# bede/kindel

Hardware: NVIDIA H100
Metric: aligned bases/sec through pileup+consensus (higher is better)
Workload: dtype int32

## Files before the change

kindel_b200/csrc/api.cu:

```cuda
#include <atomic>
#include <cstdio>
#include <cstdlib>
#include <cstring>
#include <new>

#include "kdl_common.cuh"
#include "pileup_general.cu"
#include "pileup_simple.cu"
#include "pileup_tile.cu"
#include "pileup_mask.cu"
#include "vote.cu"
#include "assemble.cu"
#include "variants.cu"
#include "select.cu"
#include "primers.cu"
#include "mates.cu"
#include "quality.cu"
#include "amplicons.cu"
#include "normalise.cu"
#include "dedup.cu"
#include "left_align.cu"

namespace {

// ... 31 lines not shown
    static std::atomic<int> done[kMaxDevices];
    const int dev = current_device();
    if (done[dev].load(std::memory_order_acquire)) return KDL_OK;
    if (cudaFuncSetAttribute(kdl::pileup_tile_kernel<kFlush, kCx>, cudaFuncAttributeMaxDynamicSharedMemorySize,
                             (int)sizeof(kdl::TileSmem<kdl::TileCfg<kCx>>)) != cudaSuccess)
        return KDL_ERR_CUDA;
    done[dev].store(1, std::memory_order_release);
    return KDL_OK;
}

inline int check_launch() {
    g_launches.fetch_add(1, std::memory_order_relaxed);
    return cudaGetLastError() == cudaSuccess ? KDL_OK : KDL_ERR_CUDA;
}
#else
inline int sm_count() { return emu::M().sm_count; }

template <int kFlush, bool kCx>
inline int ensure_tile_smem() { return KDL_OK; }

inline int check_launch() {
    g_launches.fetch_add(1, std::memory_order_relaxed);
    return emu::take_launch_error() ? KDL_ERR_CUDA : KDL_OK;
}
#endif

template <int kFlush, bool kCx>
inline int launch_tile(const kdl_batch& b, int32_t* counts, long long n_slots, long long tile_lo, long long n_tiles,
                       int split, int zero_rest, uint32_t* dirty_map, uint32_t map_after, cudaStream_t st) {
    int rc = ensure_tile_smem<kFlush, kCx>();
    if (rc != KDL_OK) return rc;
    const long long units = n_tiles * split, max_grid = (long long)sm_count() * 2;
    const long long grid = units < max_grid ? units : max_grid;
    KDL_LAUNCH((kdl::pileup_tile_kernel<kFlush, kCx>), (unsigned)grid, kdl::W_THREADS,
               sizeof(kdl::TileSmem<kdl::TileCfg<kCx>>), st,
               b, counts, n_slots, b.tile_index, tile_lo, n_tiles, split, zero_rest, dirty_map, map_after);
    return KDL_OK;
}

int depth_split(long long units, int per_sm, long long reads) {
    int split = 1;
    const long long slots = (long long)sm_count() * per_sm;
    if (units < slots) {
        long long want = (slots + units - 1) / units;
        const long long deep = reads / (units * 256);
        if (want > deep) want = deep;
        split = (int)(want < 1 ? 1 : (want > 32 ? 32 : want));
    }
    if (const char* ev = getenv("KDL_SPLIT")) { const int v = atoi(ev); if (v >= 1 && v <= 64) split = v; }
    return split;
}

int validate_batch(const kdl_batch* b) {
    if (!b || b->n_reads < 0 || b->n_contigs < 0 || b->n_hard < 0 || b->n_complex < b->n_hard)
        return KDL_ERR_INVALID_ARG;
    if (b->n_reads > 0 && (!b->ref_start || !b->seq_off || !b->l_seq || !b->seq4 ||
                           !b->contig_read_off || !b->contig_len || !b->contig_slot))
        return KDL_ERR_INVALID_ARG;
    if ((b->n_hard > 0 && !b->hard_idx) || (b->n_complex > 0 && !b->complex_idx)) return KDL_ERR_INVALID_ARG;
    if (b->reach_right < b->max_simple_len || b->reach_left < 0) return KDL_ERR_INVALID_ARG;
    return KDL_OK;
}

}

extern "C" {

int kdl_abi_version(void) { return KDL_ABI_VERSION; }

const char* kdl_status_string(int status) {
    switch (status) {
        case KDL_OK: return "ok";
        case KDL_ERR_INVALID_ARG: return "invalid argument";
        case KDL_ERR_CUDA: return "CUDA error";
        case KDL_ERR_NO_DEVICE: return "no CUDA device";
        case KDL_ERR_INDEX: return "IndexError: read walks off the contig or off its SEQ";
        case KDL_ERR_KEY: return "KeyError: base outside A,C,G,T,N in an M or S op";
        default: return "unknown status";
    }
}

int64_t kdl_launch_count(void) { return g_launches.load(std::memory_order_relaxed); }

int kdl_pileup(const kdl_batch* batch, int32_t* counts, int64_t n_slots, int32_t* ins_events,
               int32_t* err_flag, void* stream) {
    return kdl_pileup_range(batch, counts, n_slots, 0, n_slots, 0, ins_events, err_flag, stream);
}

int kdl_pileup_range(const kdl_batch* batch, int32_t* counts, int64_t n_slots, int64_t slot_lo,
                     int64_t slot_hi, int32_t flags, int32_t* ins_events, int32_t* err_flag, void* stream) {
    return kdl_pileup_range_map(batch, counts, n_slots, slot_lo, slot_hi, flags, nullptr, ins_events, err_flag, stream);
}

int kdl_pileup_range_map(const kdl_batch* batch, int32_t* counts, int64_t n_slots, int64_t slot_lo, int64_t slot_hi,
                         int32_t flags, uint32_t* dirty_map, int32_t* ins_events, int32_t* err_flag, void* stream) {
    int rc = validate_batch(batch);
    if (rc != KDL_OK) return rc;
    if (!counts || !err_flag || n_slots <= 0 || slot_lo < 0 || slot_hi > n_slots || slot_lo > slot_hi ||
        (reinterpret_cast<uintptr_t>(dirty_map) & 15))
        return KDL_ERR_INVALID_ARG;
    const bool tileable = (n_slots % KDL_TILE) == 0 && (slot_lo % KDL_TILE) == 0 && (slot_hi % KDL_TILE) == 0;
    if ((slot_lo & 3) || (slot_hi & 3)) return KDL_ERR_INVALID_ARG;
    cudaStream_t st = (cudaStream_t)stream;
    const int cap = sm_count() * 8;
    const bool has_tile_reads = batch->n_reads > batch->n_hard;
    const bool tiled = has_tile_reads && tileable && batch->reads_sorted && batch->tile_index &&
                       batch->reach_right > 0 && batch->reach_right <= KDL_FAST_MAXLEN + KDL_TILE_MAXREACH;
    const bool fresh = (flags & KDL_PILEUP_FRESH_WEIGHTS) != 0;
    const long long tile_lo = slot_lo / KDL_TILE, n_tiles = (slot_hi - slot_lo) / KDL_TILE;
    const int split = tiled && n_tiles > 0 ? depth_split(n_tiles, 2, batch->n_reads) : 1;
    bool cx_by_atomics = (batch->n_complex - batch->n_hard) * 16 < batch->n_reads;
    if (const char* ev = getenv("KDL_CX")) cx_by_atomics = !strcmp(ev, "atomics") ? true : (!strcmp(ev, "pieces") ? false : cx_by_atomics);
    const int zero_in_k1 = (tiled && split == 1 && fresh && n_tiles > 0 && (flags & KDL_PILEUP_ZERO_REST)) ? 1 : 0;
    const int zero_from = (fresh && !(tiled && split == 1)) ? 0 : 5;
    const int zero_to = ((flags & KDL_PILEUP_ZERO_REST) && !zero_in_k1) ? KDL_NCOL : 5;
    const bool zero_pass = zero_to > zero_from && slot_hi > slot_lo;
    const bool k1_stores = tiled && split == 1 && fresh && n_tiles > 0;
    const bool saturate = dirty_map && batch->n_complex > 0 && batch->n_complex * 16 >= batch->n_reads &&
                          (k1_stores || zero_pass);
    uint32_t* mark_map = saturate ? nullptr : dirty_map;
    if (zero_pass) {
        uint32_t* zmap = saturate || (zero_from <= 5 && zero_to == KDL_NCOL) ? dirty_map : nullptr;
        KDL_LAUNCH(kdl::zero_cols_kernel, sm_count() * 4, 256, 0, st, counts, n_slots, zero_from, zero_to, slot_lo,
                   slot_hi, zmap, saturate ? ~0u : 0u);
        if ((rc = check_launch()) != KDL_OK) return rc;
    }
    const uint32_t map_after = saturate && k1_stores ? ~0u : 0u;
    if (batch->n_reads == 0) return KDL_OK;
    if (tiled) {
        if (n_tiles > 0) {
            KDL_LAUNCH(kdl::tile_index_kernel, (unsigned)((n_tiles * 32 + 255) / 256), 256, 0, st, *batch, tile_lo,
                       n_tiles, batch->tile_index);
            if ((rc = check_launch()) != KDL_OK) return rc;
            const bool cx = batch->n_complex > batch->n_hard && !cx_by_atomics;
            if (split > 1) {
                rc = cx ? launch_tile<kdl::F_ATOMIC, true>(*batch, counts, n_slots, tile_lo, n_tiles, split, 0, nullptr, 0, st)
                        : launch_tile<kdl::F_ATOMIC, false>(*batch, counts, n_slots, tile_lo, n_tiles, split, 0, nullptr, 0, st);
            } else if (fresh) {
                rc = cx ? launch_tile<kdl::F_STORE, true>(*batch, counts, n_slots, tile_lo, n_tiles, 1, zero_in_k1, dirty_map,
                                                          map_after, st)
                        : launch_tile<kdl::F_STORE, false>(*batch, counts, n_slots, tile_lo, n_tiles, 1, zero_in_k1, dirty_map,
                                                           map_after, st);
            } else {
                rc = cx ? launch_tile<kdl::F_ADD, true>(*batch, counts, n_slots, tile_lo, n_tiles, 1, 0, nullptr, 0, st)
                        : launch_tile<kdl::F_ADD, false>(*batch, counts, n_slots, tile_lo, n_tiles, 1, 0, nullptr, 0, st);
            }
            if (rc != KDL_OK) return rc;
            if ((rc = check_launch()) != KDL_OK) return rc;
        }
        if (batch->n_complex > batch->n_hard && cx_by_atomics && n_tiles > 0) {
            const long long n_win = (slot_hi - slot_lo + kdl::CW_SLOTS - 1) / kdl::CW_SLOTS;
            const int wsplit = depth_split(n_win, 8, batch->n_complex - batch->n_hard);
            KDL_LAUNCH(kdl::pileup_window_kernel, (unsigned)(n_win * wsplit), kdl::CW_THREADS,
                       sizeof(int32_t) * kdl::CW_SMEM_COLS * kdl::CW_SLOTS, st, *batch, counts, n_slots, slot_lo,
                       slot_hi, wsplit, ins_events, mark_map);
            if ((rc = check_launch()) != KDL_OK) return rc;
        } else if (batch->n_complex > batch->n_hard && !cx_by_atomics) {
            KDL_LAUNCH(kdl::pileup_events_kernel, (unsigned)((batch->n_complex + 255) / 256), 256, 0, st, *batch, counts,
                       n_slots, ins_events, mark_map);
            if ((rc = check_launch()) != KDL_OK) return rc;
        }
        if (batch->n_hard > 0) {
            const int grid = grid_for(batch->n_hard, 8, cap);
            KDL_LAUNCH(kdl::pileup_general_kernel, grid, 256, 0, st, *batch, batch->hard_idx, batch->n_hard, counts,
                       n_slots, ins_events, err_flag, mark_map);
            if ((rc = check_launch()) != KDL_OK) return rc;
        }
    } else {
        if (batch->n_reads > batch->n_complex) {
            const int grid = grid_for(batch->n_reads, 8, cap);
            KDL_LAUNCH(kdl::pileup_simple_atomic_kernel, grid, 256, 0, st, *batch, counts, n_slots, err_flag);
            if ((rc = check_launch()) != KDL_OK) return rc;
        }
        if (batch->n_complex > 0) {
            const int grid = grid_for(batch->n_reads, 8, cap);
            KDL_LAUNCH(kdl::pileup_general_kernel, grid, 256, 0, st, *batch, nullptr, batch->n_reads, counts, n_slots,
                       ins_events, err_flag, mark_map);
            if ((rc = check_launch()) != KDL_OK) return rc;
        }
    }
    return KDL_OK;
}

int kdl_unmask(const kdl_batch* batch, const kdl_qmask* qmask, int32_t* counts, int64_t n_slots, void* stream) {
    int rc = validate_batch(batch);
    if (rc != KDL_OK) return rc;
    if (!qmask || !counts || n_slots <= 0 || qmask->n_reads < 0 || qmask->n_bases < 0 || qmask->n_reads > batch->n_reads)
        return KDL_ERR_INVALID_ARG;
    if (qmask->n_reads == 0) return KDL_OK;
    if (!qmask->read_idx || !qmask->off || !qmask->qpos) return KDL_ERR_INVALID_ARG;
    const long long grid = (qmask->n_reads + kdl::kQThreads - 1) / kdl::kQThreads;
    KDL_LAUNCH(kdl::unmask_kernel, (unsigned)grid, kdl::kQThreads, 0, (cudaStream_t)stream, *batch, *qmask, counts,
               n_slots);
    return check_launch();
}

int kdl_diagnose(const kdl_batch* batch, kdl_diag* diag_dev, void* stream) {
    int rc = validate_batch(batch);
    if (rc != KDL_OK) return rc;
    if (!diag_dev) return KDL_ERR_INVALID_ARG;
    cudaStream_t st = (cudaStream_t)stream;
    KDL_LAUNCH(kdl::diagnose_init_kernel, 1, 1, 0, st, diag_dev);
    if ((rc = check_launch()) != KDL_OK) return rc;
    if (batch->n_hard > 0) {
        const long long grid = (batch->n_hard + 255) / 256;
        KDL_LAUNCH(kdl::diagnose_kernel, (unsigned)grid, 256, 0, st, *batch, diag_dev);
        if ((rc = check_launch()) != KDL_OK) return rc;
    }
    KDL_LAUNCH(kdl::diagnose_final_kernel, 1, 1, 0, st, diag_dev);
    return check_launch();
}

int kdl_vote(const int32_t* counts, int64_t n_slots, int64_t min_depth_ceil, uint8_t* calls,
             void* stream) {
    if (!counts || !calls || n_slots <= 0 || (n_slots & 3)) return KDL_ERR_INVALID_ARG;
    kdl::Peers none;
    none.n = 0;
    const long long quads = n_slots / 4;
    const long long grid = (quads + 255) / 256;
    KDL_LAUNCH(kdl::vote_kernel<false>, (unsigned)grid, 256, 0, (cudaStream_t)stream,
               counts, none, n_slots, 0, n_slots, min_depth_ceil, calls, nullptr, kdl::MajorityVote{});
    return check_launch();
}

static bool valid_threshold(double t) { return t >= 0.0 && t <= 1.0; }

int kdl_vote_iupac(const int32_t* counts, int64_t n_slots, int64_t min_depth_ceil, double threshold, uint8_t* calls,
                   void* stream) {
    if (!counts || !calls || n_slots <= 0 || (n_slots & 3) || !valid_threshold(threshold)) return KDL_ERR_INVALID_ARG;
    kdl::Peers none;
    none.n = 0;
    const long long quads = n_slots / 4;
    const long long grid = (quads + 255) / 256;
    KDL_LAUNCH((kdl::vote_kernel<false, kdl::IupacVote>), (unsigned)grid, 256, 0, (cudaStream_t)stream,
               counts, none, n_slots, 0, n_slots, min_depth_ceil, calls, nullptr, kdl::IupacVote{threshold});
    return check_launch();
}

int kdl_derive(const int32_t* counts, int64_t n_slots, int32_t* out, void* stream) {
    if (!counts || !out || n_slots <= 0) return KDL_ERR_INVALID_ARG;
    const long long grid = (n_slots + 255) / 256;
    KDL_LAUNCH(kdl::derive_kernel, (unsigned)grid, 256, 0, (cudaStream_t)stream, counts, n_slots, out);
    return check_launch();
}

int kdl_vote_peers(const int32_t* const* peer_counts, int32_t n_peers, int64_t n_slots,
                   int64_t slot_lo, int64_t slot_hi, int64_t min_depth_ceil, uint8_t* calls,
                   int32_t* reduced, void* stream) {
    return kdl_vote_peers_sparse(peer_counts, nullptr, nullptr, n_peers, n_slots, slot_lo, slot_hi,
                                 min_depth_ceil, calls, reduced, stream);
}

static int make_exchange(const kdl_exchange* x, kdl::Exchange* e, int64_t n_slots) {
    if (!x || x->n_ranks < 1 || x->n_ranks > 16 || x->rank < 0 || x->rank >= x->n_ranks || !x->counter)
        return KDL_ERR_INVALID_ARG;
    e->peers.n = x->n_ranks;
    e->rank = x->rank;
    e->counter = x->counter;
    for (int p = 0; p < x->n_ranks; ++p) {
        if (!x->tables[p] || !x->calls[p] || !x->ready[p] || !x->done[p]) return KDL_ERR_INVALID_ARG;
        e->peers.tab[p] = x->tables[p];
        e->peers.lo[p] = x->foot_lo[p];
        e->peers.hi[p] = n_slots > 0 && x->foot_hi[p] > n_slots ? n_slots : x->foot_hi[p];
        if ((e->peers.lo[p] & 3) || (e->peers.hi[p] & 3)) return KDL_ERR_INVALID_ARG;
        e->calls[p] = x->calls[p];
        e->ready[p] = x->ready[p];
        e->done[p] = x->done[p];
        e->slice_lo[p] = x->slice_lo[p];
        e->slice_hi[p] = x->slice_hi[p];
        if ((x->slice_lo[p] & 3) || (x->slice_hi[p] & 3) || x->slice_hi[p] < x->slice_lo[p]) return KDL_ERR_INVALID_ARG;
    }
    e->ready_local = x->ready[x->rank];
    e->done_local = x->done[x->rank];
    return KDL_OK;
}

int kdl_exchange_signal(const kdl_exchange* x, int32_t epoch, void* stream) {
    kdl::Exchange e;
    int rc = make_exchange(x, &e, 0);
    if (rc != KDL_OK) return rc;
    KDL_LAUNCH(kdl::exchange_signal_kernel, 1, 32, 0, (cudaStream_t)stream, e, epoch);
    return check_launch();
}

int kdl_exchange_wait(const kdl_exchange* x, int32_t epoch, void* stream) {
    kdl::Exchange e;
    int rc = make_exchange(x, &e, 0);
    if (rc != KDL_OK) return rc;
    dim3 grid((unsigned)(sm_count() * 2 / x->n_ranks + 1), (unsigned)x->n_ranks);
    KDL_LAUNCH(kdl::exchange_gather_kernel, grid, 256, 0, (cudaStream_t)stream, e, epoch);
    return check_launch();
}

extern "C++" template <class Vote>
int exchange_vote(const kdl_exchange* x, int64_t n_slots, int64_t min_depth_ceil, int32_t epoch, Vote vote,
                  void* stream) {
    if (n_slots <= 0 || (n_slots & 3)) return KDL_ERR_INVALID_ARG;
    kdl::Exchange e;
    int rc = make_exchange(x, &e, n_slots);
    if (rc != KDL_OK) return rc;
    if (x->slice_hi[x->rank] > n_slots) return KDL_ERR_INVALID_ARG;
    const long long quads = (x->slice_hi[x->rank] - x->slice_lo[x->rank]) / 4;
    long long grid = (quads + 255) / 256;
    const long long cap = (long long)sm_count() * 8;
    if (grid > cap) grid = cap;
    if (grid < 1) grid = 1;
    KDL_LAUNCH(kdl::vote_exchange_kernel<Vote>, (unsigned)grid, 256, 0, (cudaStream_t)stream, e, n_slots,
// ... 698 lines not shown
```

kindel_b200/csrc/pileup_general.cu:

```cuda
#include "tile_common.cuh"

namespace kdl {

__global__ void __launch_bounds__(256)
pileup_general_kernel(kdl_batch b, const uint32_t* __restrict__ list, long long n_list, int32_t* __restrict__ counts,
                      long long n_slots, int32_t* __restrict__ ins_events, int32_t* __restrict__ err_flag,
                      uint32_t* __restrict__ dirty_map = nullptr) {
    const int lane = threadIdx.x & 31;
    const bool marks = dirty_map != nullptr && lane == 0;
    const long long warp0 = ((long long)blockIdx.x * blockDim.x + threadIdx.x) >> 5;
    const long long n_warps = ((long long)gridDim.x * blockDim.x) >> 5;
    bool bad = false;

    for (long long j = warp0; j < n_list; j += n_warps) {
        const long long r = list ? (long long)list[j] : j;
        const uint32_t lraw = (uint32_t)b.l_seq[r];
        if (!(lraw & KDL_COMPLEX)) continue;
        const int c = find_contig(b.contig_read_off, b.n_contigs, r);
        const long long L = b.contig_len[c];
        const long long base = b.contig_slot[c];
        const long long lseq = complex_len(lraw);
        const uint32_t* __restrict__ seq = b.seq4 + (size_t)b.seq_off[r];
        const uint32_t* __restrict__ blk = seq + ((lseq + 7) >> 3);
        const uint32_t c0 = 0, c1 = blk[0];
// ... 9 lines not shown
            if (op == 0 || op == 7 || op == 8) {
                for (long long k = lane; k < len; k += 32) {
                    const long long q = q_pos + k;
                    const long long idx = pyindex(r_pos + k, L);
                    if (q >= lseq || idx < 0) { bad = true; continue; }
                    const int col = nib2col(nibble_at(seq, q));
                    if (col < 0) { bad = true; continue; }
                    atomicAdd(counts + (long long)(KDL_W_A + col) * n_slots + base + idx, 1);
                }
                r_pos += len;
                q_pos += len;
            } else if (op == 1) {
                if (marks) mark_dirty_py(dirty_map, KDL_INS, 1, base, r_pos, r_pos + 1, L + 1);
                if (lane == 0) {
                    const long long idx = pyindex(r_pos, L + 1);
                    if (idx < 0) {
                        bad = true;
                    } else {
                        atomicAdd(counts + (long long)KDL_INS * n_slots + base + idx, 1);
                        if (ins_events) {
                            int4 e = make_int4((int)(base + idx), (int)r, (int)q_pos, (int)len);
                            reinterpret_cast<int4*>(ins_events)[evt] = e;
                        }
                    }
                }
                evt += 1;
                q_pos += len;
            } else if (op == 2) {
                if (marks) mark_dirty_py(dirty_map, KDL_DEL, 1, base, r_pos, r_pos + len, L + 1);
                for (long long k = lane; k < len; k += 32) {
                    const long long idx = pyindex(r_pos + k, L + 1);
                    if (idx < 0) { bad = true; continue; }
                    atomicAdd(counts + (long long)KDL_DEL * n_slots + base + idx, 1);
                }
                r_pos += len;
            } else if (op == 4) {
                if (i == c0) {
                    if (marks) {
                        mark_dirty_py(dirty_map, KDL_CLIP_ENDS, 1, base, r_pos, r_pos + 1, L + 1);
                        mark_dirty(dirty_map, KDL_CEW_A, 5, base + (r_pos - len > 0 ? r_pos - len : 0),
                                   base + (r_pos < L ? r_pos : L));
                    }
                    if (lane == 0) {
                        const long long idx = pyindex(r_pos, L + 1);
                        if (idx < 0) bad = true;
                        else atomicAdd(counts + (long long)KDL_CLIP_ENDS * n_slots + base + idx, 1);
                    }
                    for (long long g = lane; g < len; g += 32) {
                        if (g >= lseq) { bad = true; continue; }
                        const long long rel = r_pos - len + g;
                        if (rel < 0) continue;
                        if (rel >= L) { bad = true; continue; }
                        const int col = nib2col(nibble_at(seq, g));
                        if (col < 0) { bad = true; continue; }
                        atomicAdd(counts + (long long)(KDL_CEW_A + col) * n_slots + base + rel, 1);
                    }
                    q_pos += len;
                } else {
                    if (lane == 0) {
                        const long long idx = pyindex(r_pos - 1, L + 1);
                        if (idx < 0) bad = true;
                        else atomicAdd(counts + (long long)KDL_CLIP_STARTS * n_slots + base + idx, 1);
                    }
                    long long n_adv = L - r_pos;
                    n_adv = n_adv < 0 ? 0 : (n_adv > len ? len : n_adv);
                    if (marks) {
                        mark_dirty_py(dirty_map, KDL_CLIP_STARTS, 1, base, r_pos - 1, r_pos, L + 1);
                        mark_dirty_py(dirty_map, KDL_CSW_A, 5, base, r_pos, r_pos + n_adv, L);
                    }
                    for (long long k = lane; k < n_adv; k += 32) {
                        const long long q = q_pos + k;
                        const long long idx = pyindex(r_pos + k, L);
                        if (q >= lseq || idx < 0) { bad = true; continue; }
                        const int col = nib2col(nibble_at(seq, q));
                        if (col < 0) { bad = true; continue; }
                        atomicAdd(counts + (long long)(KDL_CSW_A + col) * n_slots + base + idx, 1);
                    }
                    if (n_adv < len && q_pos + n_adv >= lseq) bad = true;
                    r_pos += n_adv;
                    q_pos += n_adv;
                }
            }
        }
    }
    if (bad) atomicOr(err_flag, 1);
}

__global__ void __launch_bounds__(256)
pileup_events_kernel(kdl_batch b, int32_t* __restrict__ counts, long long n_slots, int32_t* __restrict__ ins_events,
                     uint32_t* __restrict__ dirty_map) {
    const long long j = (long long)blockIdx.x * blockDim.x + threadIdx.x;
    if (j >= b.n_complex) return;
    const long long r = (long long)b.complex_idx[j];
    const uint32_t lraw = (uint32_t)b.l_seq[r];
    if ((lraw & (KDL_COMPLEX | KDL_HARD)) != KDL_COMPLEX) return;
    const int c = find_contig(b.contig_read_off, b.n_contigs, r);
    const long long slot0 = b.contig_slot[c];
    int32_t* __restrict__ tab = counts + slot0;
    const uint32_t* __restrict__ seq = b.seq4 + (size_t)b.seq_off[r];
    const uint32_t* __restrict__ blk = seq + (((lraw & KDL_LEN_MASK) + 7) >> 3);
    const int n_ops = (int)blk[0];
    uint32_t evt = blk[1];
    const uint32_t* __restrict__ ops = blk + 2;
    long long r_pos = b.ref_start[r];
    int q_pos = 0;
    for (int o = 0; o < n_ops; ++o) {
        const uint32_t cg = ops[o];
        const int len = (int)(cg >> 4);
        const int op = (int)(cg & 0xF);
        if (op == 0 || op == 7 || op == 8) {
            r_pos += len;
            q_pos += len;
        } else if (op == 1) {
            if (dirty_map) mark_dirty(dirty_map, KDL_INS, 1, slot0 + r_pos, slot0 + r_pos + 1);
            atomicAdd(tab + (long long)KDL_INS * n_slots + r_pos, 1);
            if (ins_events)
                reinterpret_cast<int4*>(ins_events)[evt] = make_int4((int)(slot0 + r_pos), (int)r, q_pos, len);
            evt += 1;
            q_pos += len;
        } else if (op == 2) {
            if (dirty_map) mark_dirty(dirty_map, KDL_DEL, 1, slot0 + r_pos, slot0 + r_pos + len);
            for (int d = 0; d < len; ++d) atomicAdd(tab + (long long)KDL_DEL * n_slots + r_pos + d, 1);
            r_pos += len;
        } else if (op == 4) {
            if (o == 0) {
                if (dirty_map) {
                    mark_dirty(dirty_map, KDL_CLIP_ENDS, 1, slot0 + r_pos, slot0 + r_pos + 1);
                    mark_dirty(dirty_map, KDL_CEW_A, 5, slot0 + (r_pos - len > 0 ? r_pos - len : 0), slot0 + r_pos);
                }
                atomicAdd(tab + (long long)KDL_CLIP_ENDS * n_slots + r_pos, 1);
                for (int g = 0; g < len; ++g) {
                    const long long rel = r_pos - len + g;
                    if (rel >= 0) atomicAdd(tab + (long long)(KDL_CEW_A + nib2col(nibble_at(seq, g))) * n_slots + rel, 1);
                }
                q_pos += len;
            } else {
                if (dirty_map) {
                    mark_dirty(dirty_map, KDL_CLIP_STARTS, 1, slot0 + r_pos - 1, slot0 + r_pos);
                    mark_dirty(dirty_map, KDL_CSW_A, 5, slot0 + r_pos, slot0 + r_pos + len);
                }
                atomicAdd(tab + (long long)KDL_CLIP_STARTS * n_slots + r_pos - 1, 1);
                for (int d = 0; d < len; ++d)
                    atomicAdd(tab + (long long)(KDL_CSW_A + nib2col(nibble_at(seq, q_pos + d))) * n_slots + r_pos + d, 1);
                r_pos += len;
                q_pos += len;
            }
        }
    }
}

constexpr int CW_SLOTS = 1024;
constexpr int CW_THREADS = 256;
constexpr int CW_SMEM_COLS = 7;
static_assert(CW_SLOTS % KDL_TILE == 0 && CW_SLOTS % 256 == 0, "windows of whole tiles, whole map records per warp");

__device__ __forceinline__ void lower_bound2_u32(const uint32_t* __restrict__ a, long long n, uint32_t key1,
                                                 uint32_t key2, int lane, long long& r1, long long& r2) {
    long long lo[2] = {0, 0}, hi[2] = {n, n};
    const uint32_t key[2] = {key1, key2};
    while (lo[0] < hi[0] || lo[1] < hi[1]) {
        long long step[2];
        bool ge[2];
#pragma unroll
        for (int k = 0; k < 2; ++k) {
            step[k] = (hi[k] - lo[k] + 31) >> 5;
            const long long i = lo[k] + (long long)(lane + 1) * step[k] - 1;
            ge[k] = lo[k] >= hi[k] || i >= hi[k] || a[i] >= key[k];
        }
#pragma unroll
        for (int k = 0; k < 2; ++k) {
            const unsigned m = __ballot_sync(0xffffffffu, ge[k]);
            if (lo[k] >= hi[k]) continue;
            if (m == 0u) { lo[k] = hi[k]; continue; }
            const int b = __ffs(m) - 1;
            const long long nl = lo[k] + (long long)b * step[k], nh = nl + step[k] - 1;
            hi[k] = nh < hi[k] ? nh : hi[k];
            lo[k] = step[k] == 1 ? hi[k] : nl;
        }
    }
    r1 = lo[0];
    r2 = lo[1];
}

__global__ void __launch_bounds__(CW_THREADS)
pileup_window_kernel(kdl_batch b, int32_t* __restrict__ counts, long long n_slots, long long slot_lo, long long slot_hi,
                     int split, int32_t* __restrict__ ins_events, uint32_t* __restrict__ dirty_map) {
    KDL_DYNAMIC_SMEM(smem_raw);
    int* acc = reinterpret_cast<int*>(smem_raw);
    __shared__ long long range[2];
    const int tid = threadIdx.x, lane = tid & 31;
    constexpr int n_sec = CW_SMEM_COLS * (CW_SLOTS / 8);
    const long long g0 = slot_lo + (long long)(blockIdx.x / split) * CW_SLOTS;
    const long long g1 = g0 + CW_SLOTS < slot_hi ? g0 + CW_SLOTS : slot_hi;
    for (int k = tid; k < 2 * n_sec; k += CW_THREADS) reinterpret_cast<int4*>(acc)[k] = make_int4(0, 0, 0, 0);
    if (tid < 32) {
        const uint32_t lo = b.tile_index[F_IDX * (g0 / KDL_TILE)], hi = b.tile_index[F_IDX * ((g1 - 1) / KDL_TILE) + 1];
        long long ja, je;
        lower_bound2_u32(b.complex_idx, b.n_complex, lo, hi, lane, ja, je);
        if (lane == 0) {
            const int part = (int)(blockIdx.x % split);
            range[0] = ja + (je - ja) * part / split;
            range[1] = ja + (je - ja) * (part + 1) / split;
        }
    }
    __syncthreads();
    const long long j0 = range[0], j1 = range[1];
    int lg = 0;
    while (lg < 5 && ((j1 - j0) << (lg + 1)) <= CW_THREADS) ++lg;
    const int gl = tid & ((1 << lg) - 1), step = 1 << lg;
    for (long long j = j0 + (tid >> lg); j < j1; j += CW_THREADS >> lg) {
        const long long r = (long long)b.complex_idx[j];
        const uint32_t lraw = (uint32_t)b.l_seq[r];
        if ((lraw & (KDL_COMPLEX | KDL_HARD)) != KDL_COMPLEX) continue;
        const int c = find_contig(b.contig_read_off, b.n_contigs, r);
        const long long slot0 = b.contig_slot[c];
        const long long wl = g0 - slot0, wh = g1 - slot0;
        int32_t* __restrict__ tab = counts + slot0;
        const uint32_t* __restrict__ seq = b.seq4 + (size_t)b.seq_off[r];
        const uint32_t* __restrict__ blk = seq + (((lraw & KDL_LEN_MASK) + 7) >> 3);
        const int n_ops = (int)blk[0];
        uint32_t evt = blk[1];
        const uint32_t* __restrict__ ops = blk + 2;
        long long r_pos = b.ref_start[r];
        int q_pos = 0;
        const bool marks = dirty_map != nullptr && gl == 0;
        for (int o = 0; o < n_ops; ++o) {
            const uint32_t cg = ops[o];
            const int len = (int)(cg >> 4);
            const int op = (int)(cg & 0xF);
            const long long s0 = r_pos > wl ? r_pos : wl, s1 = r_pos + len < wh ? r_pos + len : wh;
            if (op == 0 || op == 7 || op == 8) {
#pragma unroll 4
                for (long long s = s0 + gl; s < s1; s += step)
                    atomicAdd(acc + (KDL_W_A + nib2col(nibble_at(seq, q_pos + (s - r_pos)))) * CW_SLOTS + (s - wl), 1);
                r_pos += len;
                q_pos += len;
            } else if (op == 1) {
                if (gl == 0 && r_pos >= wl && r_pos < wh) {
                    atomicAdd(acc + KDL_INS * CW_SLOTS + (r_pos - wl), 1);
                    if (ins_events)
                        reinterpret_cast<int4*>(ins_events)[evt] = make_int4((int)(slot0 + r_pos), (int)r, q_pos, len);
                }
                evt += 1;
                q_pos += len;
            } else if (op == 2) {
                for (long long s = s0 + gl; s < s1; s += step) atomicAdd(acc + KDL_DEL * CW_SLOTS + (s - wl), 1);
                r_pos += len;
            } else if (op == 4) {
                if (o == 0) {
                    const long long e0 = r_pos - len, c1 = r_pos < wh ? r_pos : wh;
                    long long c0 = e0 > 0 ? e0 : 0;
                    if (c0 < wl) c0 = wl;
                    if (gl == 0 && r_pos >= wl && r_pos < wh) {
                        if (marks) mark_dirty(dirty_map, KDL_CLIP_ENDS, 1, slot0 + r_pos, slot0 + r_pos + 1);
                        atomicAdd(tab + (long long)KDL_CLIP_ENDS * n_slots + r_pos, 1);
                    }
                    if (marks) mark_dirty(dirty_map, KDL_CEW_A, 5, slot0 + c0, slot0 + c1);
                    for (long long s = c0 + gl; s < c1; s += step)
                        atomicAdd(tab + (long long)(KDL_CEW_A + nib2col(nibble_at(seq, s - e0))) * n_slots + s, 1);
                    q_pos += len;
                } else {
                    if (gl == 0 && r_pos - 1 >= wl && r_pos - 1 < wh) {
                        if (marks) mark_dirty(dirty_map, KDL_CLIP_STARTS, 1, slot0 + r_pos - 1, slot0 + r_pos);
                        atomicAdd(tab + (long long)KDL_CLIP_STARTS * n_slots + r_pos - 1, 1);
                    }
                    if (marks) mark_dirty(dirty_map, KDL_CSW_A, 5, slot0 + s0, slot0 + s1);
                    for (long long s = s0 + gl; s < s1; s += step)
                        atomicAdd(tab + (long long)(KDL_CSW_A + nib2col(nibble_at(seq, q_pos + (s - r_pos)))) * n_slots + s,
                                  1);
                    r_pos += len;
                    q_pos += len;
                }
            }
        }
    }
    __syncthreads();
    for (int sec = tid; sec < n_sec; sec += CW_THREADS) {
        const int col = sec / (CW_SLOTS / 8), off = 8 * (sec % (CW_SLOTS / 8));
        const int4* sp = reinterpret_cast<const int4*>(acc) + 2 * sec;
        const int4 d0 = sp[0], d1 = sp[1];
        const bool dirty = (d0.x | d0.y | d0.z | d0.w | d1.x | d1.y | d1.z | d1.w) != 0;
        int32_t* dst = counts + (long long)col * n_slots + g0 + off;
        if (dirty && split == 1) {
            int4* p = reinterpret_cast<int4*>(dst);
            int4 v0 = p[0], v1 = p[1];
            v0.x += d0.x; v0.y += d0.y; v0.z += d0.z; v0.w += d0.w;
            v1.x += d1.x; v1.y += d1.y; v1.z += d1.z; v1.w += d1.w;
            p[0] = v0;
            p[1] = v1;
        } else if (dirty) {
            const int d[8] = {d0.x, d0.y, d0.z, d0.w, d1.x, d1.y, d1.z, d1.w};
#pragma unroll
            for (int k = 0; k < 8; ++k)
                if (d[k]) atomicAdd(dst + k, d[k]);
        }
        if (dirty_map && col >= KDL_DEL) {
            const unsigned m = __ballot_sync(0xffffffffu, dirty);
            const unsigned bits = lane < 4 ? (m >> (8 * lane)) & 0xFFu : 0u;
            if (bits)
                atomicOr(dirty_map + 4 * ((g0 + off - 8 * lane) / 64 + lane) + (col - KDL_DEL) / 4,
                         bits << (8 * ((col - KDL_DEL) % 4)));
        }
    }
}

__device__ unsigned long long diagnose_read(const kdl_batch& b, long long j) {
    const long long r = (long long)b.hard_idx[j];
    const int c = find_contig(b.contig_read_off, b.n_contigs, r);
    const long long L = b.contig_len[c];
    const long long lseq = complex_len((uint32_t)b.l_seq[r]);
    const uint32_t* __restrict__ seq = b.seq4 + (size_t)b.seq_off[r];
    const uint32_t* __restrict__ blk = seq + ((lseq + 7) >> 3);
    const uint32_t c0 = 0, c1 = blk[0];
    const uint32_t* __restrict__ cig = blk + 2;
    long long r_pos = b.ref_start[r], q_pos = 0;
#define KDL_FAIL(kind, nib)                                                                     \
    return ((unsigned long long)r << 24) | ((unsigned long long)(kind) << 20) |                 \
           ((unsigned long long)(nib) << 16) | (unsigned long long)((i - c0) > 0xFFFF ? 0xFFFF : (i - c0))
    for (uint32_t i = c0; i < c1; ++i) {
        const uint32_t cg = cig[i];
        const long long len = cg >> 4;
        const int op = cg & 0xF;
        if (op == 0 || op == 7 || op == 8) {
            for (long long k = 0; k < len; ++k) {
                if (q_pos >= lseq) KDL_FAIL(0, 0);
                if (pyindex(r_pos, L) < 0) KDL_FAIL(0, 0);
                const int nib = nibble_at(seq, q_pos);
                if (nib2col(nib) < 0) KDL_FAIL(1, nib);
                ++r_pos; ++q_pos;
            }
        } else if (op == 1) {
            if (pyindex(r_pos, L + 1) < 0) KDL_FAIL(0, 0);
            q_pos += len;
        } else if (op == 2) {
            for (long long k = 0; k < len; ++k)
                if (pyindex(r_pos + k, L + 1) < 0) KDL_FAIL(0, 0);
            r_pos += len;
        } else if (op == 4) {
            if (i == c0) {
                if (pyindex(r_pos, L + 1) < 0) KDL_FAIL(0, 0);
                for (long long g = 0; g < len; ++g) {
                    if (g >= lseq) KDL_FAIL(0, 0);
                    const long long rel = r_pos - len + g;
                    if (rel >= 0) {
                        if (rel >= L) KDL_FAIL(0, 0);
                        const int nib = nibble_at(seq, g);
                        if (nib2col(nib) < 0) KDL_FAIL(1, nib);
                    }
                }
                q_pos += len;
            } else {
                if (pyindex(r_pos - 1, L + 1) < 0) KDL_FAIL(0, 0);
                for (long long k = 0; k < len; ++k) {
                    if (q_pos >= lseq) KDL_FAIL(0, 0);
                    if (r_pos < L) {
                        if (pyindex(r_pos, L) < 0) KDL_FAIL(0, 0);
                        const int nib = nibble_at(seq, q_pos);
                        if (nib2col(nib) < 0) KDL_FAIL(1, nib);
                        ++r_pos; ++q_pos;
                    }
                }
            }
        }
    }
#undef KDL_FAIL
    return ~0ull;
}

__global__ void diagnose_init_kernel(kdl_diag* d) {
    d->status = 0; d->reserved = 0; d->read = -1; d->nibble = 0; d->op_index = 0;
    *reinterpret_cast<unsigned long long*>(&d->read) = ~0ull;
}

__global__ void __launch_bounds__(256) diagnose_kernel(kdl_batch b, kdl_diag* d) {
    const long long j = (long long)blockIdx.x * blockDim.x + threadIdx.x;
    if (j >= b.n_hard) return;
    const unsigned long long key = diagnose_read(b, j);
    if (key != ~0ull) atomicMin(reinterpret_cast<unsigned long long*>(&d->read), key);
}

__global__ void diagnose_final_kernel(kdl_diag* d) {
    const unsigned long long key = *reinterpret_cast<unsigned long long*>(&d->read);
    if (key == ~0ull) { d->status = KDL_OK; d->read = -1; return; }
    d->status = ((key >> 20) & 0xF) ? KDL_ERR_KEY : KDL_ERR_INDEX;
    d->nibble = (int)((key >> 16) & 0xF);
    d->op_index = (int)(key & 0xFFFF);
    d->read = (long long)(key >> 24);
}

}
```

Baseline: 1934 billion.

## Stage window reads via TMA bulk copies and scan l_seq instead of binary search

Rewrites the windowed complex-read pileup kernel. It scans the window's read range directly instead of binary-searching complex_idx, and it batches reads in chunks of 64. Each chunk's sequence/CIGAR blocks are staged into shared memory with mbarrier-tracked bulk async copies. When the CTA owns the window, it preloads the first four count columns from global memory so they can be written back with plain stores. Match runs are decoded eight bases at a time with a funnel shift. The aims are fewer scattered global loads, fewer search costs and fewer write-back read-modify-writes. In exchange, the kernel carries more synchronisation, uses more shared memory (capped under 48KB with a 5-block occupancy hint), and now also examines non-complex reads during the scan.

After: 1975 billion, median of 6. 2.1% higher.

```diff
diff --git a/kindel_b200/csrc/api.cu b/kindel_b200/csrc/api.cu
--- a/kindel_b200/csrc/api.cu
+++ b/kindel_b200/csrc/api.cu
@@ -207,7 +207,7 @@
             const long long n_win = (slot_hi - slot_lo + kdl::CW_SLOTS - 1) / kdl::CW_SLOTS;
             const int wsplit = depth_split(n_win, 8, batch->n_complex - batch->n_hard);
             KDL_LAUNCH(kdl::pileup_window_kernel, (unsigned)(n_win * wsplit), kdl::CW_THREADS,
-                       sizeof(int32_t) * kdl::CW_SMEM_COLS * kdl::CW_SLOTS, st, *batch, counts, n_slots, slot_lo,
+                       kdl::CW_SMEM_BYTES, st, *batch, counts, n_slots, slot_lo,
                        slot_hi, wsplit, ins_events, mark_map);
             if ((rc = check_launch()) != KDL_OK) return rc;
         } else if (batch->n_complex > batch->n_hard && !cx_by_atomics) {
diff --git a/kindel_b200/csrc/pileup_general.cu b/kindel_b200/csrc/pileup_general.cu
--- a/kindel_b200/csrc/pileup_general.cu
+++ b/kindel_b200/csrc/pileup_general.cu
@@ -185,154 +185,286 @@
 constexpr int CW_SLOTS = 1024;
 constexpr int CW_THREADS = 256;
 constexpr int CW_SMEM_COLS = 7;
+constexpr int CW_TAB_COLS = 4;
+constexpr int CW_SCAN = 2048;
+constexpr int CW_CHUNK = 64;
+constexpr int CW_STAGE_WORDS = 2048;
 static_assert(CW_SLOTS % KDL_TILE == 0 && CW_SLOTS % 256 == 0, "windows of whole tiles, whole map records per warp");
-
-__device__ __forceinline__ void lower_bound2_u32(const uint32_t* __restrict__ a, long long n, uint32_t key1,
-                                                 uint32_t key2, int lane, long long& r1, long long& r2) {
-    long long lo[2] = {0, 0}, hi[2] = {n, n};
-    const uint32_t key[2] = {key1, key2};
-    while (lo[0] < hi[0] || lo[1] < hi[1]) {
-        long long step[2];
-        bool ge[2];
-#pragma unroll
-        for (int k = 0; k < 2; ++k) {
-            step[k] = (hi[k] - lo[k] + 31) >> 5;
-            const long long i = lo[k] + (long long)(lane + 1) * step[k] - 1;
-            ge[k] = lo[k] >= hi[k] || i >= hi[k] || a[i] >= key[k];
-        }
-#pragma unroll
-        for (int k = 0; k < 2; ++k) {
-            const unsigned m = __ballot_sync(0xffffffffu, ge[k]);
-            if (lo[k] >= hi[k]) continue;
-            if (m == 0u) { lo[k] = hi[k]; continue; }
-            const int b = __ffs(m) - 1;
-            const long long nl = lo[k] + (long long)b * step[k], nh = nl + step[k] - 1;
-            hi[k] = nh < hi[k] ? nh : hi[k];
-            lo[k] = step[k] == 1 ? hi[k] : nl;
-        }
-    }
-    r1 = lo[0];
-    r2 = lo[1];
-}
-
-__global__ void __launch_bounds__(CW_THREADS)
+static_assert(CW_CHUNK % 32 == 0 && CW_CHUNK <= CW_THREADS, "whole warps of the CTA load a chunk");
+static_assert(CW_SCAN % CW_THREADS == 0 && CW_SCAN <= 65536, "whole turns of the CTA per scan, 16-bit list entries");
+static_assert((KDL_FAST_MAXLEN + 7) / 8 + 2 + KDL_TILE_MAXOPS + 6 <= CW_STAGE_WORDS,
+              "a tile-eligible read's block fits the area (only gaps between blocks make one too large)");
+
+struct CwRead {
+    long long slot0;
+    uint32_t r, lraw;
+    int32_t ref_start;
+    int32_t at;
+    uint32_t seq_off;
+    uint32_t pad;
+};
+struct CwSmem {
+    int acc[CW_SMEM_COLS * CW_SLOTS];
+    uint32_t stage[CW_STAGE_WORDS];
+    CwRead rd[CW_CHUNK];
+    uint16_t list[CW_SCAN];
+    uint64_t bar[2];
+    int n_list[2];
+    int wsum[CW_CHUNK / 32], wcnt[CW_CHUNK / 32];
+};
+constexpr size_t CW_SMEM_BYTES = sizeof(CwSmem);
+static_assert(CW_SMEM_BYTES <= 48 * 1024, "dynamic shared memory without the opt-in attribute");
+
+__device__ __forceinline__ void cw_mark_sector(uint32_t* __restrict__ dirty_map, int sec, bool dirty, long long g0,
+                                               int lane) {
+    const int col = sec / (CW_SLOTS / 8), off = 8 * (sec % (CW_SLOTS / 8));
+    if (!dirty_map || col < KDL_DEL) return;
+    const unsigned m = __ballot_sync(0xffffffffu, dirty);
+    const unsigned bits = lane < 4 ? (m >> (8 * lane)) & 0xFFu : 0u;
+    if (bits)
+        atomicOr(dirty_map + 4 * ((g0 + off - 8 * lane) / 64 + lane) + (col - KDL_DEL) / 4,
+                 bits << (8 * ((col - KDL_DEL) % 4)));
+}
+
+__global__ void __launch_bounds__(CW_THREADS, 5)
 pileup_window_kernel(kdl_batch b, int32_t* __restrict__ counts, long long n_slots, long long slot_lo, long long slot_hi,
                      int split, int32_t* __restrict__ ins_events, uint32_t* __restrict__ dirty_map) {
     KDL_DYNAMIC_SMEM(smem_raw);
-    int* acc = reinterpret_cast<int*>(smem_raw);
-    __shared__ long long range[2];
+    CwSmem& sm = *reinterpret_cast<CwSmem*>(smem_raw);
     const int tid = threadIdx.x, lane = tid & 31;
-    constexpr int n_sec = CW_SMEM_COLS * (CW_SLOTS / 8);
+    const bool own = split == 1;
     const long long g0 = slot_lo + (long long)(blockIdx.x / split) * CW_SLOTS;
     const long long g1 = g0 + CW_SLOTS < slot_hi ? g0 + CW_SLOTS : slot_hi;
-    for (int k = tid; k < 2 * n_sec; k += CW_THREADS) reinterpret_cast<int4*>(acc)[k] = make_int4(0, 0, 0, 0);
-    if (tid < 32) {
-        const uint32_t lo = b.tile_index[F_IDX * (g0 / KDL_TILE)], hi = b.tile_index[F_IDX * ((g1 - 1) / KDL_TILE) + 1];
-        long long ja, je;
-        lower_bound2_u32(b.complex_idx, b.n_complex, lo, hi, lane, ja, je);
-        if (lane == 0) {
-            const int part = (int)(blockIdx.x % split);
-            range[0] = ja + (je - ja) * part / split;
-            range[1] = ja + (je - ja) * (part + 1) / split;
-        }
-    }
+    constexpr int per_col = CW_SLOTS / 8;
+    constexpr int n_sec = CW_SMEM_COLS * per_col;
+    if (tid == 0) {
+        mbar_init(&sm.bar[0], 1);
+        mbar_init(&sm.bar[1], CW_CHUNK);
+        if (own) {
+            const uint32_t bytes = (uint32_t)(g1 - g0) * (uint32_t)sizeof(int32_t);
+            mbar_expect_tx(&sm.bar[0], CW_TAB_COLS * bytes);
+            for (int c = 0; c < CW_TAB_COLS; ++c)
+                bulk_g2s(sm.acc + c * CW_SLOTS, counts + (long long)c * n_slots + g0, bytes, &sm.bar[0]);
+        }
+    }
+    for (int k = (own ? CW_TAB_COLS * per_col : 0) + tid; k < n_sec; k += CW_THREADS) {
+        reinterpret_cast<int4*>(sm.acc)[2 * k] = make_int4(0, 0, 0, 0);
+        reinterpret_cast<int4*>(sm.acc)[2 * k + 1] = make_int4(0, 0, 0, 0);
+    }
+    const uint32_t* e0 = b.tile_index + F_IDX * (g0 / KDL_TILE);
+    const uint32_t* e1 = b.tile_index + F_IDX * ((g1 - 1) / KDL_TILE);
+    const long long lo = e0[0], hi = e1[1];
+    const int c_lo = e0[0] < e0[1] ? (int)e0[4] : 0;
+    const int c_hi = e1[0] < e1[1] ? (int)e1[5] : b.n_contigs - 1;
+    const int part = (int)(blockIdx.x % split);
+    const long long p0 = lo + (hi - lo) * part / split, p1 = lo + (hi - lo) * (part + 1) / split;
+    if (tid == 0) sm.n_list[0] = sm.n_list[1] = 0;
     __syncthreads();
-    const long long j0 = range[0], j1 = range[1];
-    int lg = 0;
-    while (lg < 5 && ((j1 - j0) << (lg + 1)) <= CW_THREADS) ++lg;
-    const int gl = tid & ((1 << lg) - 1), step = 1 << lg;
-    for (long long j = j0 + (tid >> lg); j < j1; j += CW_THREADS >> lg) {
-        const long long r = (long long)b.complex_idx[j];
-        const uint32_t lraw = (uint32_t)b.l_seq[r];
-        if ((lraw & (KDL_COMPLEX | KDL_HARD)) != KDL_COMPLEX) continue;
-        const int c = find_contig(b.contig_read_off, b.n_contigs, r);
-        const long long slot0 = b.contig_slot[c];
-        const long long wl = g0 - slot0, wh = g1 - slot0;
-        int32_t* __restrict__ tab = counts + slot0;
-        const uint32_t* __restrict__ seq = b.seq4 + (size_t)b.seq_off[r];
-        const uint32_t* __restrict__ blk = seq + (((lraw & KDL_LEN_MASK) + 7) >> 3);
-        const int n_ops = (int)blk[0];
-        uint32_t evt = blk[1];
-        const uint32_t* __restrict__ ops = blk + 2;
-        long long r_pos = b.ref_start[r];
-        int q_pos = 0;
-        const bool marks = dirty_map != nullptr && gl == 0;
-        for (int o = 0; o < n_ops; ++o) {
-            const uint32_t cg = ops[o];
-            const int len = (int)(cg >> 4);
-            const int op = (int)(cg & 0xF);
-            const long long s0 = r_pos > wl ? r_pos : wl, s1 = r_pos + len < wh ? r_pos + len : wh;
-            if (op == 0 || op == 7 || op == 8) {
-#pragma unroll 4
-                for (long long s = s0 + gl; s < s1; s += step)
-                    atomicAdd(acc + (KDL_W_A + nib2col(nibble_at(seq, q_pos + (s - r_pos)))) * CW_SLOTS + (s - wl), 1);
-                r_pos += len;
-                q_pos += len;
-            } else if (op == 1) {
-                if (gl == 0 && r_pos >= wl && r_pos < wh) {
-                    atomicAdd(acc + KDL_INS * CW_SLOTS + (r_pos - wl), 1);
-                    if (ins_events)
-                        reinterpret_cast<int4*>(ins_events)[evt] = make_int4((int)(slot0 + r_pos), (int)r, q_pos, len);
-                }
-                evt += 1;
-                q_pos += len;
-            } else if (op == 2) {
-                for (long long s = s0 + gl; s < s1; s += step) atomicAdd(acc + KDL_DEL * CW_SLOTS + (s - wl), 1);
-                r_pos += len;
-            } else if (op == 4) {
-                if (o == 0) {
-                    const long long e0 = r_pos - len, c1 = r_pos < wh ? r_pos : wh;
-                    long long c0 = e0 > 0 ? e0 : 0;
-                    if (c0 < wl) c0 = wl;
-                    if (gl == 0 && r_pos >= wl && r_pos < wh) {
-                        if (marks) mark_dirty(dirty_map, KDL_CLIP_ENDS, 1, slot0 + r_pos, slot0 + r_pos + 1);
-                        atomicAdd(tab + (long long)KDL_CLIP_ENDS * n_slots + r_pos, 1);
-                    }
-                    if (marks) mark_dirty(dirty_map, KDL_CEW_A, 5, slot0 + c0, slot0 + c1);
-                    for (long long s = c0 + gl; s < c1; s += step)
-                        atomicAdd(tab + (long long)(KDL_CEW_A + nib2col(nibble_at(seq, s - e0))) * n_slots + s, 1);
-                    q_pos += len;
-                } else {
-                    if (gl == 0 && r_pos - 1 >= wl && r_pos - 1 < wh) {
-                        if (marks) mark_dirty(dirty_map, KDL_CLIP_STARTS, 1, slot0 + r_pos - 1, slot0 + r_pos);
-                        atomicAdd(tab + (long long)KDL_CLIP_STARTS * n_slots + r_pos - 1, 1);
-                    }
-                    if (marks) mark_dirty(dirty_map, KDL_CSW_A, 5, slot0 + s0, slot0 + s1);
-                    for (long long s = s0 + gl; s < s1; s += step)
-                        atomicAdd(tab + (long long)(KDL_CSW_A + nib2col(nibble_at(seq, q_pos + (s - r_pos)))) * n_slots + s,
-                                  1);
-                    r_pos += len;
-                    q_pos += len;
-                }
-            }
-        }
-    }
-    __syncthreads();
-    for (int sec = tid; sec < n_sec; sec += CW_THREADS) {
-        const int col = sec / (CW_SLOTS / 8), off = 8 * (sec % (CW_SLOTS / 8));
-        const int4* sp = reinterpret_cast<const int4*>(acc) + 2 * sec;
-        const int4 d0 = sp[0], d1 = sp[1];
-        const bool dirty = (d0.x | d0.y | d0.z | d0.w | d1.x | d1.y | d1.z | d1.w) != 0;
-        int32_t* dst = counts + (long long)col * n_slots + g0 + off;
-        if (dirty && split == 1) {
-            int4* p = reinterpret_cast<int4*>(dst);
-            int4 v0 = p[0], v1 = p[1];
-            v0.x += d0.x; v0.y += d0.y; v0.z += d0.z; v0.w += d0.w;
-            v1.x += d1.x; v1.y += d1.y; v1.z += d1.z; v1.w += d1.w;
-            p[0] = v0;
-            p[1] = v1;
-        } else if (dirty) {
-            const int d[8] = {d0.x, d0.y, d0.z, d0.w, d1.x, d1.y, d1.z, d1.w};
-#pragma unroll
-            for (int k = 0; k < 8; ++k)
-                if (d[k]) atomicAdd(dst + k, d[k]);
-        }
-        if (dirty_map && col >= KDL_DEL) {
-            const unsigned m = __ballot_sync(0xffffffffu, dirty);
-            const unsigned bits = lane < 4 ? (m >> (8 * lane)) & 0xFFu : 0u;
-            if (bits)
-                atomicOr(dirty_map + 4 * ((g0 + off - 8 * lane) / 64 + lane) + (col - KDL_DEL) / 4,
-                         bits << (8 * ((col - KDL_DEL) % 4)));
+    uint32_t parity = 0;
+    int turn = 0;
+    bool counted = false;
+    for (long long s0 = p0; s0 < p1; s0 += CW_SCAN, turn ^= 1) {
+        uint32_t lw[CW_SCAN / CW_THREADS];
+#pragma unroll
+        for (int k = 0; k < CW_SCAN / CW_THREADS; ++k) {
+            const long long i = s0 + tid + k * CW_THREADS;
+            lw[k] = i < p1 ? (uint32_t)b.l_seq[i] : 0u;
+        }
+#pragma unroll
+        for (int k = 0; k < CW_SCAN / CW_THREADS; ++k)
+            if ((lw[k] & (KDL_COMPLEX | KDL_HARD)) == KDL_COMPLEX)
+                sm.list[atomicAdd(&sm.n_list[turn], 1)] = (uint16_t)(tid + k * CW_THREADS);
+        __syncthreads();
+        const int n_list = sm.n_list[turn];
+        counted |= n_list > 0;
+        if (tid == 0) sm.n_list[turn ^ 1] = 0;
+        for (int j = 0; j < n_list;) {
+            CwRead m;
+            bool valid = false;
+            int words = 0, incl = 0;
+            if (tid < CW_CHUNK) {
+                valid = j + tid < n_list;
+                if (valid) {
+                    const uint32_t r = (uint32_t)(s0 + sm.list[j + tid]);
+                    m.r = r;
+                    m.lraw = (uint32_t)b.l_seq[r];
+                    m.ref_start = b.ref_start[r];
+                    m.seq_off = b.seq_off[r];
+                    const long long end = (long long)r + 1 < b.n_reads ? (long long)b.seq_off[r + 1] : b.seq4_words;
+                    int cl = c_lo, ch = c_hi;
+                    while (cl < ch) {
+                        const int mid = (cl + ch) >> 1;
+                        if (b.contig_read_off[mid + 1] > (long long)r) ch = mid; else cl = mid + 1;
+                    }
+                    m.slot0 = b.contig_slot[cl];
+                    const long long wa = m.seq_off & ~3u, we = (end + 3) & ~3ll;
+                    if (we - wa <= CW_STAGE_WORDS && we <= b.seq4_words) words = (int)(we - wa);
+                }
+                incl = words;
+#pragma unroll
+                for (int d = 1; d < 32; d <<= 1) {
+                    const int t = __shfl_up_sync(0xffffffffu, incl, d);
+                    if (lane >= d) incl += t;
+                }
+                if (lane == 31) sm.wsum[tid >> 5] = incl;
+            }
+            __syncthreads();
+            if (tid < CW_CHUNK) {
+                for (int w = 0; w < (tid >> 5); ++w) incl += sm.wsum[w];
+                const bool in = valid && incl <= CW_STAGE_WORDS;
+                if (in) {
+                    m.at = words ? incl - words + (int)(m.seq_off & 3u) : -1;
+                    m.pad = 0;
+                    sm.rd[tid] = m;
+                }
+                mbar_expect_tx(&sm.bar[1], in ? (uint32_t)words * 4u : 0u);
+                if (in && words)
+                    bulk_g2s(sm.stage + (incl - words), b.seq4 + (m.seq_off & ~3u), (uint32_t)words * 4u, &sm.bar[1]);
+                const int n_in = __popc(__ballot_sync(0xffffffffu, in));
+                if (lane == 0) sm.wcnt[tid >> 5] = n_in;
+            }
+            __syncthreads();
+            int n = 0;
+#pragma unroll
+            for (int w = 0; w < CW_CHUNK / 32; ++w) n += sm.wcnt[w];
+            if (own) mbar_wait(&sm.bar[0], 0);
+            mbar_wait(&sm.bar[1], parity);
+            parity ^= 1u;
+
+            int lg = 0;
+            while (lg < 5 && (n << (lg + 1)) <= CW_THREADS) ++lg;
+            const int gl = tid & ((1 << lg) - 1), step = 1 << lg;
+            for (int i = tid >> lg; i < n; i += CW_THREADS >> lg) {
+                const CwRead& rd = sm.rd[i];
+                const uint32_t lraw = rd.lraw;
+                const long long slot0 = rd.slot0;
+                const int wn = (int)(g1 - g0);
+                const int cs = slot0 - g0 > -1 ? (int)(slot0 - g0) : -1;
+                int32_t* __restrict__ tab = counts + g0;
+                const uint32_t* __restrict__ seq = rd.at >= 0 ? sm.stage + rd.at : b.seq4 + rd.seq_off;
+                const uint32_t* __restrict__ blk = seq + (((lraw & KDL_LEN_MASK) + 7) >> 3);
+                const int n_ops = (int)blk[0];
+                uint32_t evt = blk[1];
+                const uint32_t* __restrict__ ops = blk + 2;
+                int x = (int)(slot0 + rd.ref_start - g0);
+                int q_pos = 0;
+                const bool marks = dirty_map != nullptr && gl == 0;
+                for (int o = 0; o < n_ops; ++o) {
+                    const uint32_t cg = ops[o];
+                    const int len = (int)(cg >> 4);
+                    const int op = (int)(cg & 0xF);
+                    const int s0 = x > 0 ? x : 0, s1 = x + len < wn ? x + len : wn;
+                    if (op == 0 || op == 7 || op == 8) {
+                        for (int s = s0 + 8 * gl; s < s1; s += 8 * step) {
+                            const int q = q_pos + (s - x);
+                            const uint32_t v = __funnelshift_l(seq[(q >> 3) + 1], seq[q >> 3], 4 * (q & 7));
+                            const int n8 = s1 - s < 8 ? s1 - s : 8;
+#pragma unroll
+                            for (int k = 0; k < 8; ++k)
+                                if (k < n8) atomicAdd(sm.acc + nib2col((int)((v >> (28 - 4 * k)) & 0xFu)) * CW_SLOTS + s + k, 1);
+                        }
+                        x += len;
+                        q_pos += len;
+                    } else if (op == 1) {
+                        if (gl == 0 && x >= 0 && x < wn) {
+                            atomicAdd(sm.acc + KDL_INS * CW_SLOTS + x, 1);
+                            if (ins_events)
+                                reinterpret_cast<int4*>(ins_events)[evt] = make_int4((int)(g0 + x), (int)rd.r, q_pos, len);
+                        }
+                        evt += 1;
+                        q_pos += len;
+                    } else if (op == 2) {
+                        for (int s = s0 + gl; s < s1; s += step) atomicAdd(sm.acc + KDL_DEL * CW_SLOTS + s, 1);
+                        x += len;
+                    } else if (op == 4) {
+                        if (o == 0) {
+                            const int e0 = x - len, c1 = x < wn ? x : wn;
+                            int c0 = e0 > cs ? e0 : cs;
+                            if (c0 < 0) c0 = 0;
+                            if (gl == 0 && x >= 0 && x < wn) {
+                                if (marks) mark_dirty(dirty_map, KDL_CLIP_ENDS, 1, g0 + x, g0 + x + 1);
+                                atomicAdd(tab + (long long)KDL_CLIP_ENDS * n_slots + x, 1);
+                            }
+                            if (marks) mark_dirty(dirty_map, KDL_CEW_A, 5, g0 + c0, g0 + c1);
+                            for (int s = c0 + gl; s < c1; s += step)
+                                atomicAdd(tab + (long long)(KDL_CEW_A + nib2col(nibble_at(seq, s - e0))) * n_slots + s, 1);
+                            q_pos += len;
+                        } else {
+                            if (gl == 0 && x - 1 >= 0 && x - 1 < wn) {
+                                if (marks) mark_dirty(dirty_map, KDL_CLIP_STARTS, 1, g0 + x - 1, g0 + x);
+                                atomicAdd(tab + (long long)KDL_CLIP_STARTS * n_slots + x - 1, 1);
+                            }
+                            if (marks) mark_dirty(dirty_map, KDL_CSW_A, 5, g0 + s0, g0 + s1);
+                            for (int s = s0 + gl; s < s1; s += step)
+                                atomicAdd(tab + (long long)(KDL_CSW_A + nib2col(nibble_at(seq, q_pos + (s - x)))) * n_slots + s, 1);
+                            x += len;
+                            q_pos += len;
+                        }
+                    }
+                }
+            }
+            __syncthreads();
+            j += n;
+        }
+        __syncthreads();
+    }
+
+    if (own) {
+        mbar_wait(&sm.bar[0], 0);
+        if (counted) {
+            for (int v = tid; v < CW_TAB_COLS * (CW_SLOTS / 4); v += CW_THREADS) {
+                const int col = v / (CW_SLOTS / 4), off = 4 * (v % (CW_SLOTS / 4));
+                if (g0 + off < g1)
+                    *reinterpret_cast<int4*>(counts + (long long)col * n_slots + g0 + off) =
+                        *reinterpret_cast<const int4*>(sm.acc + col * CW_SLOTS + off);
+            }
+        }
+        constexpr int kIt = ((CW_SMEM_COLS - CW_TAB_COLS) * per_col + CW_THREADS - 1) / CW_THREADS;
+        int4 d[kIt][2], v[kIt][2];
+        bool dirty[kIt];
+#pragma unroll
+        for (int k = 0; k < kIt; ++k) {
+            const int sec = CW_TAB_COLS * per_col + tid + k * CW_THREADS;
+            dirty[k] = false;
+            if (sec < n_sec) {
+                const int4* sp = reinterpret_cast<const int4*>(sm.acc) + 2 * sec;
+                d[k][0] = sp[0];
+                d[k][1] = sp[1];
+                dirty[k] = (d[k][0].x | d[k][0].y | d[k][0].z | d[k][0].w | d[k][1].x | d[k][1].y | d[k][1].z |
+                            d[k][1].w) != 0;
+                if (dirty[k]) {
+                    const int4* p = reinterpret_cast<const int4*>(counts + (long long)(sec / per_col) * n_slots + g0 +
+                                                                  8 * (sec % per_col));
+                    v[k][0] = p[0];
+                    v[k][1] = p[1];
+                }
+            }
+        }
+#pragma unroll
+        for (int k = 0; k < kIt; ++k) {
+            const int sec = CW_TAB_COLS * per_col + tid + k * CW_THREADS;
+            if (dirty[k]) {
+                int4* p = reinterpret_cast<int4*>(counts + (long long)(sec / per_col) * n_slots + g0 + 8 * (sec % per_col));
+                v[k][0].x += d[k][0].x; v[k][0].y += d[k][0].y; v[k][0].z += d[k][0].z; v[k][0].w += d[k][0].w;
+                v[k][1].x += d[k][1].x; v[k][1].y += d[k][1].y; v[k][1].z += d[k][1].z; v[k][1].w += d[k][1].w;
+                p[0] = v[k][0];
+                p[1] = v[k][1];
+            }
+            if (sec < n_sec) cw_mark_sector(dirty_map, sec, dirty[k], g0, lane);
+        }
+    } else {
+        for (int sec = tid; sec < n_sec; sec += CW_THREADS) {
+            const int4* sp = reinterpret_cast<const int4*>(sm.acc) + 2 * sec;
+            const int4 d0 = sp[0], d1 = sp[1];
+            const int dv[8] = {d0.x, d0.y, d0.z, d0.w, d1.x, d1.y, d1.z, d1.w};
+            int32_t* dst = counts + (long long)(sec / per_col) * n_slots + g0 + 8 * (sec % per_col);
+            bool dirty = false;
+#pragma unroll
+            for (int k = 0; k < 8; ++k) {
+                if (dv[k]) atomicAdd(dst + k, dv[k]);
+                dirty |= dv[k] != 0;
+            }
+            cw_mark_sector(dirty_map, sec, dirty, g0, lane);
         }
     }
 }
```
